# AI4quantum/qiskit-gym

Hardware: AMD Instinct MI355X
Metric: env-steps/sec (whole node), CliffordGym 16q x 65536 envs/GPU; bit-exact vs CPU (higher is better)
Workload: dtype u32

## Files before the change

### qiskit_gym_amd/csrc/kernels_pauli_tile.hip

```cpp
#include <algorithm>
#include <cstdlib>
#include <cstring>

#include "device_common.hpp"
#include "pauli_common.hpp"

namespace qg {

static uint64_t ptile_program(const qg_gate &g) {
    const uint32_t a = (uint32_t)g.q0, b = g.kind >= QG_CX ? (uint32_t)g.q1 : (uint32_t)g.q0;
    struct Mop { uint32_t kind; bool swapped; };
    Mop mops[3] = {{M_NOP, false}, {M_NOP, false}, {M_NOP, false}};
    switch (g.kind) {
    case QG_H: mops[0] = {M_H, false}; break;
    case QG_S: mops[0] = {M_S, false}; break;
    case QG_SDG: mops[0] = mops[1] = mops[2] = {M_S, false}; break;
    case QG_SX: mops[0] = {M_SX, false}; break;
    case QG_SXDG: mops[0] = mops[1] = mops[2] = {M_SX, false}; break;
    case QG_CX: mops[0] = {M_CNOT, false}; break;
    case QG_CZ: mops[0] = {M_H, true}; mops[1] = {M_CNOT, false}; mops[2] = {M_H, true}; break;
    case QG_SWAP: mops[0] = {M_CNOT, false}; mops[1] = {M_CNOT, true}; mops[2] = {M_CNOT, false}; break;
    }
    uint32_t row[4] = {1, 2, 4, 8};
    auto X = [&](bool second) -> uint32_t & { return row[(second && a != b) ? 2 : 0]; };
// ... 1112 lines not shown
    const uint64_t w = row < N ? wx : wz;
    const uint32_t extra = row < N ? ex : ez;
    if (a.format == QG_FMT_PACKED) {
        reinterpret_cast<uint64_t *>(a.out)[env * a.out_stride + row] = w;
        return;
    }
    if (a.format == QG_FMT_I64) {
        int64_t *o = reinterpret_cast<int64_t *>(a.out) + env * a.out_stride + (uint64_t)row * cols;
        for (uint32_t c = 0; c < D; ++c) o[c] = (int64_t)((w >> c) & 1ull);
        for (uint32_t c = D; c < cols; ++c) o[c] = (int64_t)((extra >> (c - D)) & 1u);
    } else {
        int8_t *o = reinterpret_cast<int8_t *>(a.out) + env * a.out_stride + (uint64_t)row * cols;
        for (uint32_t c = 0; c < D; ++c) o[c] = (int8_t)((w >> c) & 1ull);
        for (uint32_t c = D; c < cols; ++c) o[c] = (int8_t)((extra >> (c - D)) & 1u);
    }
}


struct PTGenArgs {
    StepArgs s;
    const uint8_t *pairs;
    const uint32_t *dvals;
    const uint32_t *doff;
    const uint8_t *cx_pairs;
    uint32_t nd, n_cx;
    uint64_t seed;
    uint32_t difficulty, pauli_difficulty, max_paulis;
    float decay;
    int32_t depth_value;
    uint32_t only_done;
    const uint32_t *list;
    uint32_t *list_count;
    uint32_t n_pairs;
    uint32_t gen_grid;
    uint32_t tree_grid;
    uint32_t *count_out;
    uint32_t tree;
    unsigned long long *tree_kclk;
    const uint64_t *mask;
    uint32_t mask_words, mask_epoch;
    uint32_t *count_pub;
};
constexpr uint32_t PT_CX_LDS = plan::PAULI_CX_LDS;
using plan::pauli_tree_takes;

constexpr uint64_t PT_STREAM_LABELS = 0x7061756Cull, PT_STREAM_TABLEAU = 0x7461626Cull;
struct PTStream {
    uint64_t seed, env, k;
    const uint64_t *pre = nullptr;
    uint32_t n_pre = 0;
    __device__ uint64_t at(uint64_t i) const { return (pre && i < n_pre) ? pre[i] : rng_draw(seed, env, i); }
    __device__ uint64_t next() { return at(k++); }
    __device__ uint32_t range(uint32_t n) { return (uint32_t)__umul64hi(next(), (uint64_t)n); }
    __device__ float f32() { return (float)(next() >> 40) * (1.0f / 16777216.0f); }
};

struct PTGenTables {
    alignas(4) uint8_t cx[2 * PT_CX_LDS];
    uint32_t dvals[32], doff[33];
    alignas(4) uint8_t pairs[2 * 496];
};
__device__ inline bool pt_gen_tables_load(const PTGenArgs &ga, PTGenTables &t) {
    const bool cx_in_lds = ga.n_cx <= PT_CX_LDS;
    const uint32_t nd = ga.nd < 32u ? ga.nd : 32u;
    const uint32_t n_pairs = ga.n_pairs < 496u ? ga.n_pairs : 496u;
    const uint32_t cx_words = cx_in_lds ? (2u * ga.n_cx + 3u) / 4u : 0u, pair_words = (2u * n_pairs + 3u) / 4u;
    const uint32_t *cxw = reinterpret_cast<const uint32_t *>(ga.cx_pairs), *pw = reinterpret_cast<const uint32_t *>(ga.pairs);
    uint32_t *t_cx = reinterpret_cast<uint32_t *>(t.cx), *t_pairs = reinterpret_cast<uint32_t *>(t.pairs);
    constexpr uint32_t CX_PER = 8, PAIR_PER = 4;
    uint32_t cv[CX_PER], pv[PAIR_PER];
    const uint32_t dv = threadIdx.x < nd ? ga.dvals[threadIdx.x] : 0u, df = threadIdx.x <= nd ? ga.doff[threadIdx.x] : 0u;
#pragma unroll
    for (uint32_t k = 0; k < CX_PER; ++k) {
        const uint32_t i = threadIdx.x + k * blockDim.x;
// ... 223 lines not shown
    s.bad = (uint32_t)__ballot(q_lane && (X != ix || Z != iz));
    uint32_t n_removed = 0, fault = 0;
    uint64_t rem_pos[(RM + 7) / 8];
#pragma unroll
    for (int i = 0; i < (RM + 7) / 8; ++i) rem_pos[i] = 0;
    pt_clean<NQ, RM>(s, n_removed, fault, SolLog{nullptr, 0}, rem_pos);
    const bool solved = pt_solved<NQ, RM>(s);
    if (q_lane) L::store_qubit(tile, le, lane, X, Z);
    if constexpr (L::COMPACT) {
        if (q_lane) pt_store_xz<NQ, RM>(tile, le, s, lane);
        if (lane == 0) pt_store_rotmeta<NQ, RM>(tile, le, s, true);
    } else {
        if (lane == 0) pt_store_rotations<NQ, RM>(tile, le, s, ~0u, ~0u, true);
    }
    if (lane != 0) return;
    pt_store_meta<NQ, RM>(tile, le, s);
    a.depth[env] = ga.depth_value;
    a.success[env] = (uint8_t)solved;
    a.reward[env] = solved ? 1.0f : 0.0f;
    a.done[env] = (uint8_t)(ga.depth_value == 0 || solved);
    a.inverted[env] = 0;
    a.error[env] = fault;
    a.sol_len[env * 2] = 0;
    a.sol_len[env * 2 + 1] = 0;
    if (a.layers) {
        const LayerRec lay = layer_rec(a.layers, env, (2 * N + 2));
        for (uint32_t i = 0; i < 2 * N; ++i) lay[i] = -1;
        lay[2 * N] = 0;
        lay[2 * N + 1] = 0;
    }
}

template <int NQ, int RM>
__device__ __forceinline__ bool ptile_generate_body(const PTGenArgs &ga, uint32_t vblock) {
    const StepArgs &a = ga.s;
    __shared__ uint64_t lds_tab[2 * NQ][QG_WAVE];
    __shared__ PTGenTables tb;
    const uint64_t tid = (uint64_t)vblock * QG_WAVE + threadIdx.x;
    __shared__ uint32_t mask_part[64 + 1 + 5];
    uint32_t count = ga.list ? ga.list_count[0] : 0u;
    if (ga.mask) {
        const bool published = ga.tree != 0;
        count = published ? *ga.count_pub : 0u;
        if (published && (pauli_tree_takes(count, ga.difficulty, a.B, ga.n_cx) || (tid & ~(uint64_t)(QG_WAVE - 1)) >= count)) return false;
        DoneMaskShare share;
        done_mask_load<64>(ga.mask, a.B, ga.mask_words, share);
        count = *done_mask_hint(ga.mask, a.B) != ga.mask_epoch ? 0u : done_mask_scan<64>(share, mask_part);
        if ((tid & ~(uint64_t)(QG_WAVE - 1)) >= count) return false;
    } else if (ga.list && ((ga.tree && pauli_tree_takes(count, ga.difficulty, a.B, ga.n_cx)) || (tid & ~(uint64_t)(QG_WAVE - 1)) >= count)) {
        return false;
    }
    const bool cx_in_lds = pt_gen_tables_load(ga, tb);
    __builtin_amdgcn_fence(__ATOMIC_RELEASE, "wavefront");
    __builtin_amdgcn_wave_barrier();
    uint64_t env = tid;
    if (ga.mask) {
        if (tid >= count) return true;
        env = done_mask_nth<64>(ga.mask, ga.mask_words, mask_part, (uint32_t)tid);
    } else if (ga.list) {
        if (tid >= count) return true;
        env = ga.list[tid];
    } else {
        if (env >= a.B) return true;
        if (ga.only_done && !a.done[env]) return true;
    }
    const uint32_t L = threadIdx.x & (QG_WAVE - 1);
    const uint32_t N = a.N;
    const uint64_t base_seed = ga.seed + QG_CLOCK_SEED_STRIDE * clock_of(a.clock);
    PTStream rng{base_seed ^ PT_STREAM_LABELS, a.env_base + env, 0};
    PTState<NQ, RM> s;
    (void)pt_gen_labels<NQ, RM>(ga, tb, rng, s, N);

#pragma unroll
    for (int j = 0; j < NQ; ++j) {
        lds_tab[j][L] = (uint32_t)j < N ? 1ull << j : 0ull;
        lds_tab[NQ + j][L] = (uint32_t)j < N ? (1ull << N) << j : 0ull;
    }
    if (ga.difficulty != 0 && ga.n_cx != 0) {
        const uint64_t tseed = base_seed ^ PT_STREAM_TABLEAU;
        for (uint32_t it0 = 0; it0 < ga.difficulty; it0 += 4) {
            uint64_t d1[4], d2[4];
#pragma unroll
            for (uint32_t j = 0; j < 4; ++j) {
                d1[j] = rng_draw(tseed, rng.env, 2ull * (it0 + j));
                d2[j] = rng_draw(tseed, rng.env, 2ull * (it0 + j) + 1ull);
            }
#pragma unroll
            for (uint32_t j = 0; j < 4; ++j) {
                if (it0 + j >= ga.difficulty) break;
                const float r = (float)(d1[j] >> 40) * (1.0f / 16777216.0f);
                if (r > 0.3f) {
                    const uint32_t k = (uint32_t)__umul64hi(d2[j], (uint64_t)ga.n_cx);
                    const uint32_t q0 = cx_in_lds ? tb.cx[2 * k] : ga.cx_pairs[2 * k], q1 = cx_in_lds ? tb.cx[2 * k + 1] : ga.cx_pairs[2 * k + 1];
                    const uint64_t x0 = lds_tab[q0][L], z1 = lds_tab[NQ + q1][L];
                    lds_tab[q1][L] ^= x0;
                    lds_tab[NQ + q0][L] ^= z1;
                } else if (r > 0.15f) {
                    const uint32_t q = (uint32_t)__umul64hi(d2[j], (uint64_t)N);
                    const uint64_t x = lds_tab[q][L], z = lds_tab[NQ + q][L];
                    lds_tab[q][L] = z;
                    lds_tab[NQ + q][L] = x;
                } else {
                    const uint32_t q = (uint32_t)__umul64hi(d2[j], (uint64_t)N);
                    lds_tab[NQ + q][L] ^= lds_tab[q][L];
                }
            }
        }
    }
#pragma unroll
    for (int j = 0; j < NQ; ++j) {
        s.X[j] = lds_tab[j][L];
        s.Z[j] = lds_tab[NQ + j][L];
    }
    pt_gen_finish<NQ, RM>(ga, s, env, N);
    return true;
}
template <int NQ, int RM>
__global__ __launch_bounds__(64) void ptile_generate_kernel(PTGenArgs ga) {
    KernelClock kclk(ga.s.kclk, ga.s.kclk_waves);
    if (ga.mask && ga.tree) {
        const uint32_t count = *ga.count_pub;
        if (!count || pauli_tree_takes(count, ga.difficulty, ga.s.B, ga.n_cx)) return;
    }
    const uint32_t total = (uint32_t)((ga.s.B + QG_WAVE - 1) / QG_WAVE);
    for (uint32_t vblock = blockIdx.x; vblock < total; vblock += gridDim.x) {
        if (!ptile_generate_body<NQ, RM>(ga, vblock)) break;
        __builtin_amdgcn_wave_barrier();
    }
}

constexpr uint32_t PT_TREE_THREADS = QG_TREE_THREADS + QG_WAVE;
template <int NQ, int RM>
__global__ __launch_bounds__(PT_TREE_THREADS) void ptile_reset_tree_kernel(PTGenArgs ga) {
    KernelClock kclk(ga.tree_kclk, ga.s.kclk_waves);
    const StepArgs &a = ga.s;
    constexpr int R = 2 * NQ;
    __shared__ uint64_t prod[4][64];
    __shared__ RowopMasks64 tree_gates[4][QG_WAVE];
    __shared__ PTGenTables tb;
    __shared__ uint64_t rows_out[64];
    __shared__ uint64_t pre_draws[QG_TREE_THREADS];
    uint32_t count;
    __shared__ uint32_t mask_part[PT_TREE_THREADS + 2 + PT_TREE_THREADS / 64];
    DoneMaskShare share;
    uint32_t opaque_zero, first_v = 0;
    asm("v_mov_b32 %0, 0" : "=v"(opaque_zero));
    if (ga.mask) {
        first_v = done_mask_hint(ga.mask, a.B)[opaque_zero];
        done_mask_load<PT_TREE_THREADS>(ga.mask, a.B, ga.mask_words, share);
    } else {
        first_v = ga.list_count[opaque_zero];
    }
    asm volatile("" ::: "memory");
    (void)pt_gen_tables_load(ga, tb);
    if (ga.mask) {
        count = (uint32_t)__builtin_amdgcn_readfirstlane((int)first_v) != ga.mask_epoch ? 0u : done_mask_scan<PT_TREE_THREADS>(share, mask_part);
        if (blockIdx.x == 0 && threadIdx.x == 0) *ga.count_pub = count;
    } else {
        count = (uint32_t)__builtin_amdgcn_readfirstlane((int)first_v);
    }
    if (ga.count_out && blockIdx.x == 0 && threadIdx.x == 0) *ga.count_out = count;
    if (threadIdx.x == 0) phase_stamp(ga.tree_kclk, a.kclk_waves, 0);
    if (!pauli_tree_takes(count, ga.difficulty, a.B, ga.n_cx)) return;
    const uint32_t N = a.N, lane = threadIdx.x & (QG_WAVE - 1), wave = threadIdx.x >> 6;
    __shared__ uint32_t prod_ready[4];
    if (threadIdx.x < 4u) prod_ready[threadIdx.x] = 0u;
    uint32_t prod_seq = 0;
    for (uint32_t item = blockIdx.x; item < count; item += gridDim.x) {
    if (item != blockIdx.x) __syncthreads();
    const uint64_t env = !ga.mask ? ga.list[item]
                       : item == blockIdx.x ? done_mask_find<PT_TREE_THREADS>(ga.mask, ga.mask_words, share, mask_part, item)
                                            : done_mask_nth<PT_TREE_THREADS>(ga.mask, ga.mask_words, mask_part, item);
    const uint64_t base_seed = ga.seed + QG_CLOCK_SEED_STRIDE * clock_of(a.clock), renv = a.env_base + env;
    PTStream rng{base_seed ^ PT_STREAM_LABELS, renv, 0};
    if (threadIdx.x < QG_TREE_THREADS) pre_draws[threadIdx.x] = rng_draw(rng.seed, rng.env, threadIdx.x);
    __syncthreads();
    rng.pre = pre_draws;
    rng.n_pre = QG_TREE_THREADS;
    if ((threadIdx.x & 63u) == 0 && (wave == 0u || wave == 4u)) phase_stamp(ga.tree_kclk, a.kclk_waves, wave == 0u ? 1u : 2u);
    if (wave == 4u) {
        PTState<NQ, RM> s;
        (void)pt_gen_labels_wave<NQ, RM>(ga, tb, rng, s, N);
        phase_stamp(ga.tree_kclk, a.kclk_waves, 3);
        __syncthreads();
        phase_stamp(ga.tree_kclk, a.kclk_waves, 5);
        pt_gen_finish_wave<NQ, RM>(ga, s, env, N, rows_out);
        phase_stamp(ga.tree_kclk, a.kclk_waves, 6);
        continue;
    }
    const uint32_t n_cx = ga.n_cx;
    const uint8_t *cx = tb.cx;
    const uint64_t tseed = base_seed ^ PT_STREAM_TABLEAU;
    uint64_t row = 0;
    const bool finisher = scramble_tree64_ops<R>(
        ga.difficulty, row, prod, tree_gates,
        [N](uint32_t k) -> uint64_t { const uint32_t j = k < (uint32_t)NQ ? k : k - (uint32_t)NQ; return j < N ? (k < (uint32_t)NQ ? 1ull << j : (1ull << N) << j) : 0ull; },
        [=](uint32_t it) -> uint32_t {
            const uint64_t d1 = rng_draw(tseed, renv, 2ull * it), d2 = rng_draw(tseed, renv, 2ull * it + 1ull);
// ... 164 lines not shown
    ObsArgs a;
    memset(&a, 0, sizeof a);
    a.state = v->state;
    a.B = v->B;
    a.N = v->N;
    a.D = 2 * v->N;
    a.obs_rows = 2 * v->N;
    a.obs_cols = 2 * v->N + (uint32_t)std::max(v->cfg.max_rotations, 1);
    a.format = QG_FMT_U8;
    if (!a.B) return hipSuccess;
    PTObsArgs pa;
    fill_obs(v, a, pa);
    hipLaunchKernelGGL(ptile_rowwords_kernel, dim3(grid_for(a.B * 2ull * a.N / 2, 256)), dim3(256), 0, s, pa, reinterpret_cast<uint64_t *>(out_dev));
    return hipGetLastError();
}

hipError_t ptile_observe_typed(qg_vec *v, void *out_dev, int out_dtype, hipStream_t s) {
    ObsArgs a;
    memset(&a, 0, sizeof a);
    a.state = v->state;
    a.B = v->B;
    a.N = v->N;
    a.D = 2 * v->N;
    a.obs_rows = 2 * v->N;
    a.obs_cols = 2 * v->N + (uint32_t)std::max(v->cfg.max_rotations, 1);
    a.format = QG_FMT_U8;
    if (!a.B) return hipSuccess;
    return ptile_dense_via_words(v, a, out_dev, out_dtype, s);
}


template <int NQ, int RM>
static hipError_t pt_launch_generate(const PTGenArgs &pa, hipStream_t s) {
    if (pa.tree) {
        const uint64_t blocks = pa.tree_grid;
        if (blocks) hipLaunchKernelGGL((ptile_reset_tree_kernel<NQ, RM>), dim3((unsigned)blocks), dim3(PT_TREE_THREADS), 0, s, pa);
    }
    const unsigned all = grid_for(pa.s.B, 64);
    hipLaunchKernelGGL((ptile_generate_kernel<NQ, RM>), dim3(pa.gen_grid && pa.gen_grid < all ? pa.gen_grid : all), dim3(64), 0, s, pa);
    return hipGetLastError();
}
static hipError_t ptile_generate(const qg_vec *v, const PTGenArgs &pa, hipStream_t s) { PT_DISPATCH(pt_launch_generate) }

int ptile_reset_seeded(qg_vec *v, uint64_t seed, bool only_done, hipStream_t s, bool from_mask) {
    const uint32_t n = v->N;
    if (!v->d_gen_tables) {
        std::vector<uint8_t> cx;
        std::vector<std::vector<uint32_t>> adj(n);
        for (const qg_gate &g : v->gates)
            if (g.kind == QG_CX) {
                cx.push_back((uint8_t)g.q0);
                cx.push_back((uint8_t)g.q1);
                auto add = [&](uint32_t a, uint32_t b) { if (std::find(adj[a].begin(), adj[a].end(), b) == adj[a].end()) adj[a].push_back(b); };
                add((uint32_t)g.q0, (uint32_t)g.q1);
                add((uint32_t)g.q1, (uint32_t)g.q0);
            }
        std::vector<std::vector<int>> dist(n, std::vector<int>(n, -1));
        for (uint32_t st = 0; st < n; ++st) {
            std::vector<uint32_t> q{st};
            dist[st][st] = 0;
            for (size_t h = 0; h < q.size(); ++h)
                for (uint32_t w : adj[q[h]])
                    if (dist[st][w] < 0) { dist[st][w] = dist[st][q[h]] + 1; q.push_back(w); }
        }
        std::vector<uint8_t> pairs;
        std::vector<uint32_t> dvals, doff;
        for (int d = 1; d < (int)n; ++d) {
            const size_t before = pairs.size();
            for (uint32_t a = 0; a < n; ++a)
                for (uint32_t b = a + 1; b < n; ++b)
                    if (dist[a][b] == d) { pairs.push_back((uint8_t)a); pairs.push_back((uint8_t)b); }
            if (pairs.size() != before) { dvals.push_back((uint32_t)d); doff.push_back((uint32_t)(before / 2)); }
// ... 19 lines not shown
    a.state = v->state;
    a.depth = v->depth;
    a.reward = v->reward;
    a.done = v->done;
    a.success = v->success;
    a.inverted = v->inverted;
    a.error = v->error;
    a.sol_len = v->sol_len;
    a.layers = v->layers;
    a.B = v->B;
    a.N = n;
    const uint8_t *base = reinterpret_cast<const uint8_t *>(v->d_gen_tables);
    ga.dvals = reinterpret_cast<const uint32_t *>(base + v->gen_off[0]);
    ga.doff = reinterpret_cast<const uint32_t *>(base + v->gen_off[1]);
    ga.pairs = base + v->gen_off[2];
    ga.cx_pairs = base + v->gen_off[3];
    ga.nd = v->gen_nd;
    ga.n_cx = v->gen_ncx;
    ga.n_pairs = v->gen_npairs;
    ga.seed = seed;
    a.clock = v->clock_dev;
    a.env_base = v->env_base;
    ga.difficulty = (uint32_t)v->difficulty;
    ga.pauli_difficulty = (uint32_t)(v->difficulty / std::max(v->cfg.pauli_diff_scale, 1));
    ga.max_paulis = v->plan.rmax_generate;
    ga.decay = v->cfg.num_qubits_decay;
    const int64_t d = (int64_t)v->cfg.depth_slope * v->difficulty;
    ga.depth_value = (int32_t)std::min<int64_t>(d, v->cfg.max_depth);
    ga.only_done = only_done ? 1u : 0u;
    if (only_done && from_mask && v->done_mask[0]) {
        ga.mask = v->done_mask[v->dl.cur()];
        ga.mask_words = (uint32_t)done_mask_words(v->B);
        ga.mask_epoch = v->dl.epoch();
        ga.count_pub = v->mask_count;
        ga.tree = (ga.difficulty >= plan::TREE_MIN_DRAWS && v->B / 32u >= 1u && pauli_tree_takes(1u, ga.difficulty, v->B, ga.n_cx)) ? 1u : 0u;
    } else if (only_done && v->done_list && v->B > QG_COMPACT_MIN_ENVS) {
        HIP_TRY(compact_done(v->done, v->B, v->done_list, v->done_list + v->B, s));
        ga.list = v->done_list;
        ga.list_count = v->done_list + v->B;
        ga.tree = (ga.difficulty >= plan::TREE_MIN_DRAWS && v->B / 32u >= 1u && pauli_tree_takes(1u, ga.difficulty, v->B, ga.n_cx)) ? 1u : 0u;
    }
    if (ga.tree) {
        ga.tree_grid = reset_tree_grid(v, (uint32_t)(v->B / 32u));
        ga.gen_grid = reset_second_grid(v, [](uint32_t count, const qg_vec *h) -> bool {
            return pauli_tree_takes(count, (uint32_t)h->difficulty, h->B, h->gen_ncx);
        });
        ga.count_out = v->count_seen;
        ga.tree_kclk = kernel_clock_slot(v);
    }
    a.kclk = kernel_clock_slot(v);
    a.kclk_waves = v->kclk_waves;
    HIP_TRY(ptile_generate(v, ga, s));
    return QG_OK;
}

int ptile_upload(qg_vec *v, const HostNet &h, bool do_clean, int32_t depth_value, hipStream_t s) {
    const uint32_t N = v->N, NQ = v->plan.pt_nq, RM = v->plan.pt_rm;
    const bool compact = v->plan.pauli_compact;
    const size_t QB = compact ? 768 : 1024, RB = compact ? 512 : 1024, tile_bytes = NQ * QB + RM * RB + (RM > 16 ? 3072 : 1024);
    std::vector<uint8_t> img(v->plan.state_bytes, 0);
    for (uint64_t e = 0; e < v->B; ++e) {
        uint8_t *tile = img.data() + (e >> 6) * tile_bytes;
        const uint32_t lane = (uint32_t)(e & 63);
        for (uint32_t q = 0; q < N; ++q) {
            const uint64_t x = h.tab[(e * N + q) * 2], z = h.tab[(e * N + q) * 2 + 1];
            if (compact) {
                uint32_t g[3] = {(uint32_t)x, ((uint32_t)(x >> 32) & 0xFFFFu) | ((uint32_t)z << 16), (uint32_t)(z >> 16)};
                memcpy(tile + q * QB + lane * 12, g, 12);
            } else {
                uint32_t g[4] = {(uint32_t)x, (uint32_t)(x >> 32), (uint32_t)z, (uint32_t)(z >> 32)};
                memcpy(tile + q * QB + lane * 16, g, 16);
            }
        }
        if (compact) {
            uint8_t *rb = tile + NQ * QB;
            auto byte_at = [&](uint32_t b) -> uint8_t & { return rb[(b >> 3) * RB + lane * 8 + (b & 7u)]; };
            uint32_t wp[5] = {0, 0, 0, 0, 0}, plo = 0, phi = 0;
            for (uint32_t k = 0; k < v->plan.rmax; ++k) {
                const PauliRot &r = h.rot[e * v->plan.rmax + k];
                for (uint32_t q = 0; q < N; ++q) {
                    byte_at(2 * q) |= (uint8_t)(((r.x >> q) & 1u) << k);
                    byte_at(2 * q + 1) |= (uint8_t)(((r.z >> q) & 1u) << k);
                }
// ... 55 lines not shown
```

### qiskit_gym_amd/csrc/qgym_api.cpp

```cpp
#include <atomic>
#include <hip/hip_runtime.h>

#include <algorithm>
#include <cmath>
#include <cctype>
#include <cstdarg>
#include <cstdio>
#include <cstdlib>
#include <cstring>
#include <memory>
#include <string>
#include <vector>

#include "pauli_common.hpp"

namespace qg {

static thread_local std::string g_err;

int set_error(int code, const char *fmt, ...) {
    char buf[512];
    va_list ap;
    va_start(ap, fmt);
    vsnprintf(buf, sizeof buf, fmt, ap);
// ... 206 lines not shown
    while (b < e && isspace((unsigned char)name[b])) ++b;
    while (e > b && isspace((unsigned char)name[e - 1])) --e;
    name = name.substr(b, e - b);
    std::string key = name;
    for (auto &ch : key) ch = (char)tolower((unsigned char)ch);
    for (size_t i = 0; i < n; ++i)
        if (idx[i] < 0) return set_error(QG_ERR_TYPE, "Gate indices must be non-negative integers (usize)");
    static const char *one_q[] = {"h", "s", "sdg", "sx", "sxdg"};
    static const char *two_q[] = {"cx", "cz", "swap"};
    for (int k = 0; k < 5; ++k)
        if (key == one_q[k]) {
            if (n != 1) return set_error(QG_ERR_INVALID, "Gate `%s` expects 1 index, got %zu", name.c_str(), n);
            out->kind = k;
            out->q0 = (int32_t)idx[0];
            out->q1 = 0;
            return QG_OK;
        }
    for (int k = 0; k < 3; ++k)
        if (key == two_q[k]) {
            if (n != 2) return set_error(QG_ERR_INVALID, "Gate `%s` expects 2 indices, got %zu", name.c_str(), n);
            out->kind = 5 + k;
            out->q0 = (int32_t)idx[0];
            out->q1 = (int32_t)idx[1];
            return QG_OK;
        }
    return set_error(QG_ERR_INVALID, "Unknown gate name `%s`. Allowed: H, S, Sdg, SX, SXdg, CX, CZ, SWAP", name.c_str());
}


static int vec_free_buffers(qg_vec *v) {
    void *ptrs[] = {v->state, v->own_depth ? v->depth : nullptr, v->own_reward ? v->reward : nullptr,
                    v->own_done ? v->done : nullptr, v->own_success ? v->success : nullptr, v->inverted, v->own_error ? v->error : nullptr, v->sol,
                    v->sol_len, v->layers, v->d_gates, v->d_descs, v->scratch, v->d_prog,
                    v->d_qubit_perms, v->d_act_perms, v->perm_idx, v->d_gen_tables, v->d_nonsymp, v->bad, v->done_list, v->done_list_alt, v->done_list_spare, v->done_mask[0], v->done_mask[1], v->mask_count, v->d_rowops, v->embed_dump, v->host_in, v->host_obs, v->fault_scratch, v->d_twist_obs, v->twist_words};
    for (void *p : ptrs)
        if (p) (void)hipFree(p);
    drop_graphs(v);
    if (v->capture_stream) (void)hipStreamDestroy(v->capture_stream);
    if (v->fault_word) (void)hipHostFree(v->fault_word);
    if (v->count_seen) (void)hipHostFree(v->count_seen);
    return 0;
}

static int drop_done_list(qg_vec *v, hipStream_t s) { return zero_list_length(v, v->done_list, v->dl.drop(), s); }

static void fill_init_args(const qg_vec *v, InitArgs &a) {
    memset(&a, 0, sizeof a);
    a.tree_grid = plan::tree_grid(v->B);
    a.state = v->state;
    a.depth = v->depth;
    a.reward = v->reward;
    a.done = v->done;
    a.success = v->success;
    a.inverted = v->inverted;
    a.error = v->error;
    a.sol_len = v->sol_len;
    a.layers = v->layers;
    a.layers_len = v->layers_len;
    a.gates = v->d_gates;
    a.B = v->B;
    a.D = v->plan.D;
    a.N = v->N;
    a.num_actions = (uint32_t)v->gates.size();
    a.clock = v->clock_dev;
    a.env_base = v->env_base;
    a.bad = v->bad;
    a.rowops = v->d_rowops;
// ... 105 lines not shown
#define HIP_TRY_V(expr)                                                                            \
    do {                                                                                           \
        hipError_t _e = (expr);                                                                    \
        if (_e != hipSuccess) {                                                                    \
            (void)hipGetLastError();                                                               \
            return fail(set_error(QG_ERR_DEVICE, "%s failed: %s", #expr, hipGetErrorString(_e)));  \
        }                                                                                          \
    } while (0)

    HIP_TRY_V(hipMalloc(&p->state, hp.state_bytes));
    HIP_TRY_V(hipMemset(p->state, 0, hp.state_bytes));
    HIP_TRY_V(hipMalloc(&p->depth, sizeof(int32_t) * batch));
    HIP_TRY_V(hipMalloc(&p->reward, sizeof(float) * batch));
    HIP_TRY_V(hipMalloc(&p->done, batch));
    HIP_TRY_V(hipMalloc(&p->success, batch));
    HIP_TRY_V(hipMalloc(&p->inverted, batch));
    if (hp.has_bad)
        HIP_TRY_V(hipMalloc(&p->bad, plan::bad_word_bytes(hp) * batch));
    if (hp.has_done_list) {
        HIP_TRY_V(hipMalloc(&p->done_list, sizeof(uint32_t) * (batch + 2)));
        HIP_TRY_V(hipMemset(p->done_list + batch, 0, 2 * sizeof(uint32_t)));
    }
    if (hp.has_done_list && plan::is_tile(hp)) {
        HIP_TRY_V(hipMalloc(&p->done_list_spare, sizeof(uint32_t) * (batch + 2)));
        HIP_TRY_V(hipMemset(p->done_list_spare + batch, 0, 2 * sizeof(uint32_t)));
    }
    if (plan::reset_step_fusable(hp)) {
        HIP_TRY_V(hipMalloc(&p->done_list_alt, sizeof(uint32_t) * (batch + 2)));
        HIP_TRY_V(hipMemset(p->done_list_alt + batch, 0, 2 * sizeof(uint32_t)));
    }
    if (hp.has_done_list) {
        HIP_TRY_V(hipHostMalloc((void **)&p->count_seen, sizeof(uint32_t), hipHostMallocMapped));
        *p->count_seen = 0xFFFFFFFFu;
        if (hp.layout != LAYOUT_TILE) {
            HIP_TRY_V(hipMalloc(&p->mask_count, 2 * sizeof(uint32_t)));
            HIP_TRY_V(hipMemset(p->mask_count, 0, 2 * sizeof(uint32_t)));
        }
        for (auto &m : p->done_mask) {
            HIP_TRY_V(hipMalloc(&m, done_mask_bytes(batch)));
            HIP_TRY_V(hipMemset(m, 0, done_mask_bytes(batch)));
        }
    }
    HIP_TRY_V(hipMalloc(&p->error, sizeof(uint32_t) * batch));
    HIP_TRY_V(hipMalloc(&p->sol_len, sizeof(int32_t) * 2 * batch));
    if (cfg->track_solution) {
        p->sol_cap = (uint32_t)std::max(cfg->max_depth, 1);
        if (hp.layout == LAYOUT_PAULI) p->sol_cap += hp.rmax;
        HIP_TRY_V(hipMalloc(&p->sol, sizeof(uint32_t) * (size_t)p->sol_cap * batch));
    }
    if (layers) {
        p->layers_len = 2 * N + 2;
        HIP_TRY_V(hipMalloc(&p->layers, sizeof(int32_t) * (size_t)p->layers_len * (((size_t)batch + 63) & ~(size_t)63)));
    }
    (void)device_compute_units(device);
    uint32_t group_bytes[plan::GROUP_TABLE_DWORDS] = {};
    if (hp.layout == LAYOUT_TILE) plan::gate_group_bytes(&table[0].ops, sizeof(GateEntry) / sizeof(uint32_t), n_gates, hp.has_z, group_bytes);
    HIP_TRY_V(hipMalloc(&p->d_gates, sizeof(GateEntry) * table.size() + sizeof group_bytes));
    HIP_TRY_V(hipMalloc(&p->d_descs, sizeof(uint32_t) * descs.size()));
    HIP_TRY_V(hipMemcpy(p->d_gates, table.data(), sizeof(GateEntry) * table.size(), hipMemcpyHostToDevice));
    HIP_TRY_V(hipMemcpy(p->d_gates + n_gates, group_bytes, sizeof group_bytes, hipMemcpyHostToDevice));
    HIP_TRY_V(hipMemcpy(p->d_descs, descs.data(), sizeof(uint32_t) * descs.size(), hipMemcpyHostToDevice));
    if (plan::is_tile(hp)) {
        std::vector<uint32_t> rowops(table.size(), 0u);
        auto slot = [&](uint32_t row) { return hp.has_z ? (row < N ? 2 * row : 2 * (row - N) + 1) : row; };
        for (size_t i = 0; i < n_gates; ++i) {
            const uint32_t ops = gate_ops(cfg->env_kind, gates[i], N);
            uint32_t out = 0;
            for (int k = 0; k < 2; ++k) {
                const uint32_t op = (ops >> (14 * k)) & 0x3FFFu, type = (op >> 12) & 3u;
                if (type != OP_NONE) out |= make_op(type, slot(op & 63u), slot((op >> 6) & 63u)) << (14 * k);
// ... 230 lines not shown
        HIP_TRY(hipStreamSynchronize(s));
    }
    return QG_OK;
}

static int do_reset(qg_vec *v, const int32_t *actions_dev, uint64_t seed, hipStream_t s, bool only_done = false) {
    QG_ON_DEVICE(v);
    const bool trusted = v->dl.enter(session_of(s));
    if (int rc = only_done ? QG_OK : drop_done_list(v, s)) return rc;
    if (only_done && v->plan.layout == LAYOUT_PAULI) return ptile_reset_seeded(v, seed, true, s, v->dl.pauli_reset_consumes(trusted));
    if (v->plan.layout == LAYOUT_PAULI) {
        if (actions_dev) return set_error(QG_ERR_UNSUPPORTED, "PauliEnv reset draws a whole target, not `difficulty` actions: use qg_vec_reset(seed) or qg_vec_pauli_reset_from");
        return pauli_reset_seeded(v, seed, s);
    }
    if (v->gates.empty() && v->difficulty)
        return set_error(QG_ERR_PANIC, "reset with an empty gateset (the reference panics in Uniform::new(0, 0))");
    InitArgs ia;
    fill_reset_done_args(v, seed, ia);
    ia.actions = actions_dev;
    ia.only_done = only_done ? 1u : 0u;
    if (only_done && v->done_list) {
        const DoneListState::Consume use = v->dl.reset_consumes(trusted);
        if (use.compact) HIP_TRY(compact_done(v->done, v->B, v->done_list, v->done_list + v->B, s));
        ia.list = v->done_list;
        ia.list_count = v->done_list + v->B;
        if (plan::is_tile(v->plan) && v->count_seen) {
            ia.count_out = v->count_seen;
            ia.tree_grid = reset_tree_grid(v, plan::tree_grid(v->B));
        }
        if (use.mask && v->done_mask[0]) {
            ia.mask = v->done_mask[v->dl.cur()];
            ia.mask_words = (uint32_t)done_mask_words(v->B);
            ia.mask_epoch = v->dl.epoch();
            ia.count_pub = v->mask_count;
        }
        ia.coop = plan::reset_coop_allowed(actions_dev != nullptr, v->B, v->d_rowops != nullptr) ? 1u : 0u;
        ia.flags_current = 1u;
        if (v->plan.layout == LAYOUT_TILE) ia.dense = v->dense;
        if (v->done_list_spare) ia.zero_count = v->done_list_spare + v->B;
    }
    if (!only_done) v->maybe_nonsymplectic = false;
    HIP_TRY(launch_init(v, ia, s));
    if (ia.zero_count) std::swap(v->done_list, v->done_list_spare);
    if (v->dense && !ia.dense) return dense_refresh(v, s);
    return QG_OK;
}

int qg_vec_set_clock(qg_vec *v, const uint64_t *clock_dev) {
    if (!v) return set_error(QG_ERR_INVALID, "null argument");
    QG_ON_DEVICE(v);
    HIP_TRY(hipDeviceSynchronize());
    v->clock_dev = clock_dev;
    drop_graphs(v);
    return QG_OK;
}

int qg_vec_set_kernel_clock(qg_vec *v, uint64_t *slots_dev, size_t n_slots, uint32_t waves_per_slot) {
    if (!v || (n_slots && (!slots_dev || !waves_per_slot))) return set_error(QG_ERR_INVALID, "null argument");
    if ((uintptr_t)slots_dev & 15u) return set_error(QG_ERR_INVALID, "kernel clock slots must be 16-byte aligned");
    drop_graphs(v);
    v->kclk = n_slots ? reinterpret_cast<unsigned long long *>(slots_dev) : nullptr;
    v->kclk_cap = n_slots;
    v->kclk_waves = n_slots ? waves_per_slot : 0u;
    v->kclk_next = 0;
    return QG_OK;
}

// ... 605 lines not shown
        hipMemcpy(len.data(), v->sol_len, len.size() * sizeof(int32_t), hipMemcpyDeviceToHost) != hipSuccess ||
        hipMemcpy(log.data(), v->sol, log.size() * sizeof(uint32_t), hipMemcpyDeviceToHost) != hipSuccess) {
        (void)hipGetLastError();
        return set_error(QG_ERR_DEVICE, "solution copy failed");
    }
    for (size_t e = 0; e < v->B; ++e) lens[e] = (int64_t)decode_solution(v, log.data() + e, v->B, &len[2 * e], out ? out + e * cap : nullptr, cap);
    return QG_OK;
}

}

namespace qg {
uint64_t session_of(hipStream_t s) {
    hipStreamCaptureStatus cs = hipStreamCaptureStatusNone;
    unsigned long long id = 0;
    if (s) (void)hipStreamGetCaptureInfo(s, &cs, &id);
    return cs == hipStreamCaptureStatusNone ? 0ull : (id ? (uint64_t)id : ~0ull);
}
int zero_list_length(const qg_vec *v, uint32_t *list, bool needed, hipStream_t s) {
    if (needed) HIP_TRY(hipMemsetAsync(list + v->B, 0, 2 * sizeof(uint32_t), s));
    return QG_OK;
}
int bind_error(qg_vec *v, uint32_t *error_dev) {
    if (!v || !error_dev) return set_error(QG_ERR_INVALID, "null argument");
    QG_ON_DEVICE(v);
    HIP_TRY(hipDeviceSynchronize());
    HIP_TRY(hipMemcpy(error_dev, v->error, sizeof(uint32_t) * v->B, hipMemcpyDefault));
    if (v->own_error) (void)hipFree(v->error);
    v->error = error_dev;
    v->own_error = false;
    drop_graphs(v);
    return QG_OK;
}
uint32_t reset_second_grid(const qg_vec *v, bool is_tree_list_of_that_length(uint32_t, const qg_vec *)) {
    const uint32_t seen = v->count_seen ? *(volatile const uint32_t *)v->count_seen : 0xFFFFFFFFu;
    return (seen != 0xFFFFFFFFu && (seen == 0 || is_tree_list_of_that_length(seen, v))) ? 32u : 0u;
}

int dense_refresh(qg_vec *v, hipStream_t s) {
    ObsArgs oa;
    fill_obs_args(v, oa, v->dense, QG_FMT_U8, (size_t)v->plan.D * v->plan.D);
    HIP_TRY(launch_export(v, oa, s));
    return QG_OK;
}
void fill_reset_done_args(const qg_vec *v, uint64_t seed, InitArgs &ia) {
    fill_init_args(v, ia);
    ia.mode = 2;
    ia.n_draws = (uint32_t)v->difficulty;
    ia.seed = seed;
    ia.only_done = 1u;
    ia.depth_value = (int32_t)std::min<int64_t>((int64_t)v->cfg.depth_slope * v->difficulty, v->cfg.max_depth);
}
}
```

### qiskit_gym_amd/csrc/qgym_host.hpp

```cpp
#pragma once

#include <string.h>
#include <string>
#include <vector>

#include "qgym_done_list.hpp"
#include "qgym_internal.hpp"
#include "qgym_plan.hpp"

namespace qg {

struct GraphKey {
    const void *actions;
    const void *coins;
    const void *rewards;
    const void *dones;
    size_t T;
    int dtype;
    size_t period;
    uint32_t flags;
    uint64_t env_base;
    const void *dense;
    bool operator==(const GraphKey &o) const {
        return actions == o.actions && coins == o.coins && rewards == o.rewards && dones == o.dones && T == o.T &&
// ... 58 lines not shown
    unsigned long long *kclk = nullptr;
    size_t kclk_cap = 0;
    uint32_t kclk_waves = 0;
    mutable size_t kclk_next = 0;

    void *state = nullptr;
    int32_t *depth = nullptr;
    float *reward = nullptr;
    uint8_t *done = nullptr;
    uint8_t *success = nullptr;
    uint8_t *inverted = nullptr;
    uint32_t *error = nullptr;
    uint32_t *sol = nullptr;
    int32_t *sol_len = nullptr;
    int32_t *layers = nullptr;
    qg::GateEntry *d_gates = nullptr;
    uint32_t *d_descs = nullptr;
    uint32_t sol_cap = 0;
    uint32_t layers_len = 0;
    void *scratch = nullptr;
    size_t scratch_bytes = 0;
    void *host_in = nullptr;
    void *host_obs = nullptr;
    size_t host_obs_bytes = 0;
    uint32_t *count_seen = nullptr;
    uint32_t *fault_word = nullptr;
    uint32_t *fault_scratch = nullptr;
    uint32_t *bad = nullptr;
    uint32_t *d_rowops = nullptr;
    uint32_t *done_list = nullptr;
    uint32_t *done_list_alt = nullptr;
    uint32_t *done_list_spare = nullptr;
    uint64_t *done_mask[2] = {nullptr, nullptr};
    uint32_t *mask_count = nullptr;
    qg::DoneListState dl;
    int8_t *dense = nullptr;
    uint32_t *d_nonsymp = nullptr;
    void *embed_dump = nullptr;
    bool maybe_nonsymplectic = false;
    bool own_reward = true, own_done = true, own_success = true, own_depth = true;
    bool own_error = true;

    void *d_prog = nullptr;
    void *d_gen_tables = nullptr;
    uint32_t gen_nd = 0, gen_ncx = 0, gen_npairs = 0, gen_off[4] = {0, 0, 0, 0};
    uint8_t *d_qubit_perms = nullptr;
    int32_t *d_act_perms = nullptr;
    uint32_t *perm_idx = nullptr;
    const int32_t *perm_in = nullptr;
    uint32_t n_perms = 0;
    bool perm_draw = false;
    uint64_t observe_counter = 0;

    bool twists_done = false;
    std::vector<std::vector<int64_t>> obs_perms, act_perms;
    int32_t *d_twist_obs = nullptr;
    void *twist_words = nullptr;
    size_t twist_words_bytes = 0;

    std::vector<qg::CachedGraph> graphs;
    hipStream_t capture_stream = nullptr;
};

namespace qg {
inline bool same_ctor(const qg_vec *a, const qg_vec *b) {
    return a->device == b->device && memcmp(&a->cfg, &b->cfg, sizeof a->cfg) == 0 && a->gates.size() == b->gates.size() &&
           (a->gates.empty() || memcmp(a->gates.data(), b->gates.data(), a->gates.size() * sizeof(qg_gate)) == 0);
}
int ensure_scratch(qg_vec *v, size_t bytes);
inline void destroy_graph(CachedGraph &g) {
    if (g.exec) (void)hipGraphExecDestroy(g.exec);
    if (g.graph) (void)hipGraphDestroy(g.graph);
}
inline void drop_graphs(qg_vec *v) {
    for (auto &g : v->graphs) destroy_graph(g);
    v->graphs.clear();
}
uint64_t session_of(hipStream_t s);
int zero_list_length(const qg_vec *v, uint32_t *list, bool needed, hipStream_t s);
void fill_step_args(const qg_vec *v, StepArgs &a);
int bind_error(qg_vec *v, uint32_t *error_dev);
uint32_t reset_second_grid(const qg_vec *v, bool is_tree_list_of_that_length(uint32_t, const qg_vec *));
uint32_t reset_tree_grid(const qg_vec *v, uint32_t most);
unsigned long long *kernel_clock_slot(const qg_vec *v);
int dense_refresh(qg_vec *v, hipStream_t s);
void fill_reset_done_args(const qg_vec *v, uint64_t seed, InitArgs &ia);
void compute_qubit_and_action_perms(uint32_t N, const std::vector<qg_gate> &gates, std::vector<std::vector<int64_t>> &qubit_perms,
                                    std::vector<std::vector<int64_t>> &act_perms);
void build_twists(const qg_vec *v, std::vector<std::vector<int64_t>> &obs_perms, std::vector<std::vector<int64_t>> &act_perms);
int twist_expand_impl(const void *packed_dev, int word_bytes, uint64_t batch, uint32_t rows, uint32_t cols, const int32_t *obs_perms_dev,
                      uint32_t n_twists, const int32_t *twist_idx_dev, void *out_dev, int out_dtype, hipStream_t s);
int twist_words_impl(const void *packed_dev, int word_bytes, uint64_t batch, uint32_t rows, uint32_t cols, const int32_t *obs_perms_dev,
                     uint32_t n_twists, const int32_t *twist_idx_dev, uint64_t *out_dev, uint32_t rows_out, hipStream_t s);
int pauli_alloc(qg_vec *v);
int pauli_init_identity(qg_vec *v, hipStream_t s);
int pauli_set_state(qg_vec *v, const void *states, int format, size_t stride, int on_device, hipStream_t s);
int pauli_reset_from(qg_vec *v, const uint8_t *tableaus, const char *labels, const int32_t *n_rot, hipStream_t s);
int pauli_reset_seeded(qg_vec *v, uint64_t seed, hipStream_t s);
hipError_t pauli_step(const qg_vec *v, const StepArgs &a, hipStream_t s);
hipError_t pauli_export(const qg_vec *v, const ObsArgs &a, hipStream_t s);
}
```

Baseline: 26.11 billion.

## Fold per-env generate walk into reset tree kernel, dropping second launch

When the tree path is selected, the reset tree kernel now also handles the case where the tree is not taken: it walks the done list or mask itself, using a union of LDS between the tree scratch and a per-wave tableau, instead of publishing a count and launching a second generate kernel. This removes one kernel launch per reset, the count_pub global handshake and the host-side second-grid heuristic. The cost is a heavier tree kernel with more LDS and a waves_per_eu attribute, and the walk runs only on the first wave of blocks up to count/64, which may give less parallelism than the old separate generate grid.

After: 26.08 billion, median of 2. No clear change (-0.1%).

```diff
diff --git a/qiskit_gym_amd/csrc/kernels_pauli_tile.hip b/qiskit_gym_amd/csrc/kernels_pauli_tile.hip
--- a/qiskit_gym_amd/csrc/kernels_pauli_tile.hip
+++ b/qiskit_gym_amd/csrc/kernels_pauli_tile.hip
@@ -1168,14 +1168,12 @@
     const uint32_t *list;
     uint32_t *list_count;
     uint32_t n_pairs;
-    uint32_t gen_grid;
     uint32_t tree_grid;
     uint32_t *count_out;
     uint32_t tree;
     unsigned long long *tree_kclk;
     const uint64_t *mask;
     uint32_t mask_words, mask_epoch;
-    uint32_t *count_pub;
 };
 constexpr uint32_t PT_CX_LDS = plan::PAULI_CX_LDS;
 using plan::pauli_tree_takes;
@@ -1465,38 +1463,8 @@
 }
 
 template <int NQ, int RM>
-__device__ __forceinline__ bool ptile_generate_body(const PTGenArgs &ga, uint32_t vblock) {
+__device__ __forceinline__ void ptile_generate_env(const PTGenArgs &ga, const PTGenTables &tb, uint64_t (*lds_tab)[QG_WAVE], bool cx_in_lds, uint64_t env) {
     const StepArgs &a = ga.s;
-    __shared__ uint64_t lds_tab[2 * NQ][QG_WAVE];
-    __shared__ PTGenTables tb;
-    const uint64_t tid = (uint64_t)vblock * QG_WAVE + threadIdx.x;
-    __shared__ uint32_t mask_part[64 + 1 + 5];
-    uint32_t count = ga.list ? ga.list_count[0] : 0u;
-    if (ga.mask) {
-        const bool published = ga.tree != 0;
-        count = published ? *ga.count_pub : 0u;
-        if (published && (pauli_tree_takes(count, ga.difficulty, a.B, ga.n_cx) || (tid & ~(uint64_t)(QG_WAVE - 1)) >= count)) return false;
-        DoneMaskShare share;
-        done_mask_load<64>(ga.mask, a.B, ga.mask_words, share);
-        count = *done_mask_hint(ga.mask, a.B) != ga.mask_epoch ? 0u : done_mask_scan<64>(share, mask_part);
-        if ((tid & ~(uint64_t)(QG_WAVE - 1)) >= count) return false;
-    } else if (ga.list && ((ga.tree && pauli_tree_takes(count, ga.difficulty, a.B, ga.n_cx)) || (tid & ~(uint64_t)(QG_WAVE - 1)) >= count)) {
-        return false;
-    }
-    const bool cx_in_lds = pt_gen_tables_load(ga, tb);
-    __builtin_amdgcn_fence(__ATOMIC_RELEASE, "wavefront");
-    __builtin_amdgcn_wave_barrier();
-    uint64_t env = tid;
-    if (ga.mask) {
-        if (tid >= count) return true;
-        env = done_mask_nth<64>(ga.mask, ga.mask_words, mask_part, (uint32_t)tid);
-    } else if (ga.list) {
-        if (tid >= count) return true;
-        env = ga.list[tid];
-    } else {
-        if (env >= a.B) return true;
-        if (ga.only_done && !a.done[env]) return true;
-    }
     const uint32_t L = threadIdx.x & (QG_WAVE - 1);
     const uint32_t N = a.N;
     const uint64_t base_seed = ga.seed + QG_CLOCK_SEED_STRIDE * clock_of(a.clock);
@@ -1546,15 +1514,44 @@
         s.Z[j] = lds_tab[NQ + j][L];
     }
     pt_gen_finish<NQ, RM>(ga, s, env, N);
+}
+
+template <int NQ, int RM>
+__device__ __forceinline__ bool ptile_generate_body(const PTGenArgs &ga, uint32_t vblock) {
+    const StepArgs &a = ga.s;
+    __shared__ uint64_t lds_tab[2 * NQ][QG_WAVE];
+    __shared__ PTGenTables tb;
+    const uint64_t tid = (uint64_t)vblock * QG_WAVE + threadIdx.x;
+    __shared__ uint32_t mask_part[64 + 1 + 5];
+    uint32_t count = ga.list ? ga.list_count[0] : 0u;
+    if (ga.mask) {
+        DoneMaskShare share;
+        done_mask_load<64>(ga.mask, a.B, ga.mask_words, share);
+        count = *done_mask_hint(ga.mask, a.B) != ga.mask_epoch ? 0u : done_mask_scan<64>(share, mask_part);
+        if ((tid & ~(uint64_t)(QG_WAVE - 1)) >= count) return false;
+    } else if (ga.list && (tid & ~(uint64_t)(QG_WAVE - 1)) >= count) {
+        return false;
+    }
+    const bool cx_in_lds = pt_gen_tables_load(ga, tb);
+    __builtin_amdgcn_fence(__ATOMIC_RELEASE, "wavefront");
+    __builtin_amdgcn_wave_barrier();
+    uint64_t env = tid;
+    if (ga.mask) {
+        if (tid >= count) return true;
+        env = done_mask_nth<64>(ga.mask, ga.mask_words, mask_part, (uint32_t)tid);
+    } else if (ga.list) {
+        if (tid >= count) return true;
+        env = ga.list[tid];
+    } else {
+        if (env >= a.B) return true;
+        if (ga.only_done && !a.done[env]) return true;
+    }
+    ptile_generate_env<NQ, RM>(ga, tb, lds_tab, cx_in_lds, env);
     return true;
 }
 template <int NQ, int RM>
 __global__ __launch_bounds__(64) void ptile_generate_kernel(PTGenArgs ga) {
     KernelClock kclk(ga.s.kclk, ga.s.kclk_waves);
-    if (ga.mask && ga.tree) {
-        const uint32_t count = *ga.count_pub;
-        if (!count || pauli_tree_takes(count, ga.difficulty, ga.s.B, ga.n_cx)) return;
-    }
     const uint32_t total = (uint32_t)((ga.s.B + QG_WAVE - 1) / QG_WAVE);
     for (uint32_t vblock = blockIdx.x; vblock < total; vblock += gridDim.x) {
         if (!ptile_generate_body<NQ, RM>(ga, vblock)) break;
@@ -1563,16 +1560,51 @@
 }
 
 constexpr uint32_t PT_TREE_THREADS = QG_TREE_THREADS + QG_WAVE;
-template <int NQ, int RM>
-__global__ __launch_bounds__(PT_TREE_THREADS) void ptile_reset_tree_kernel(PTGenArgs ga) {
+struct PTTreeLds {
+    uint64_t prod[4][64];
+    RowopMasks64 tree_gates[4][QG_WAVE];
+    uint64_t rows_out[64];
+    uint64_t pre_draws[QG_TREE_THREADS];
+    uint32_t prod_ready[4];
+};
+template <int NQ>
+union PTResetLds {
+    PTTreeLds tree;
+    uint64_t walk_tab[2 * NQ][QG_WAVE];
+};
+using PTGenArgsSegment = const __attribute__((address_space(4))) PTGenArgs *;
+template <int NQ, int RM>
+__device__ __noinline__ void ptile_tree_walk(PTGenArgsSegment args, uint32_t count, const PTGenTables *tb_lds, const uint32_t *mask_part_lds,
+                                             uint64_t (*tab_lds)[QG_WAVE]) {
+    const uint64_t args_v = (uint64_t)args;
+    const uint32_t args_lo = (uint32_t)__builtin_amdgcn_readfirstlane((int)(uint32_t)args_v), args_hi = (uint32_t)__builtin_amdgcn_readfirstlane((int)(uint32_t)(args_v >> 32));
+    const PTGenArgs &ga = *(const PTGenArgs *)(PTGenArgsSegment)(((uint64_t)args_hi << 32) | args_lo);
+    const PTGenTables &tb = *(const PTGenTables *)(const __attribute__((address_space(3))) PTGenTables *)tb_lds;
+    const uint32_t *mask_part = (const uint32_t *)(const __attribute__((address_space(3))) uint32_t *)mask_part_lds;
+    uint64_t (*tab)[QG_WAVE] = (uint64_t (*)[QG_WAVE])(__attribute__((address_space(3))) uint64_t (*)[QG_WAVE])tab_lds;
+    count = (uint32_t)__builtin_amdgcn_readfirstlane((int)count);
+    const uint32_t vblocks = (count + QG_WAVE - 1u) / QG_WAVE;
+    for (uint32_t vblock = blockIdx.x; vblock < vblocks; vblock += gridDim.x) {
+        const uint32_t i = vblock * QG_WAVE + threadIdx.x;
+        if (i < count) {
+            const uint64_t env = ga.mask ? done_mask_nth<PT_TREE_THREADS>(ga.mask, ga.mask_words, mask_part, i) : ga.list[i];
+            ptile_generate_env<NQ, RM>(ga, tb, tab, true , env);
+        }
+        __builtin_amdgcn_wave_barrier();
+    }
+}
+template <int NQ, int RM>
+__global__ __launch_bounds__(PT_TREE_THREADS) __attribute__((amdgpu_waves_per_eu(RM > 16 ? 4 : 5))) void ptile_reset_tree_kernel(PTGenArgs ga) {
     KernelClock kclk(ga.tree_kclk, ga.s.kclk_waves);
     const StepArgs &a = ga.s;
     constexpr int R = 2 * NQ;
-    __shared__ uint64_t prod[4][64];
-    __shared__ RowopMasks64 tree_gates[4][QG_WAVE];
+    __shared__ PTResetLds<NQ> lds;
+    uint64_t (&prod)[4][64] = lds.tree.prod;
+    RowopMasks64 (&tree_gates)[4][QG_WAVE] = lds.tree.tree_gates;
+    uint64_t (&rows_out)[64] = lds.tree.rows_out;
+    uint64_t (&pre_draws)[QG_TREE_THREADS] = lds.tree.pre_draws;
+    uint32_t (&prod_ready)[4] = lds.tree.prod_ready;
     __shared__ PTGenTables tb;
-    __shared__ uint64_t rows_out[64];
-    __shared__ uint64_t pre_draws[QG_TREE_THREADS];
     uint32_t count;
     __shared__ uint32_t mask_part[PT_TREE_THREADS + 2 + PT_TREE_THREADS / 64];
     DoneMaskShare share;
@@ -1588,15 +1620,18 @@
     (void)pt_gen_tables_load(ga, tb);
     if (ga.mask) {
         count = (uint32_t)__builtin_amdgcn_readfirstlane((int)first_v) != ga.mask_epoch ? 0u : done_mask_scan<PT_TREE_THREADS>(share, mask_part);
-        if (blockIdx.x == 0 && threadIdx.x == 0) *ga.count_pub = count;
     } else {
         count = (uint32_t)__builtin_amdgcn_readfirstlane((int)first_v);
     }
     if (ga.count_out && blockIdx.x == 0 && threadIdx.x == 0) *ga.count_out = count;
     if (threadIdx.x == 0) phase_stamp(ga.tree_kclk, a.kclk_waves, 0);
-    if (!pauli_tree_takes(count, ga.difficulty, a.B, ga.n_cx)) return;
+    if (!pauli_tree_takes(count, ga.difficulty, a.B, ga.n_cx)) {
+        if (blockIdx.x >= (count + QG_WAVE - 1u) / QG_WAVE) return;
+        __syncthreads();
+        if (threadIdx.x < QG_WAVE) ptile_tree_walk<NQ, RM>((PTGenArgsSegment)__builtin_amdgcn_kernarg_segment_ptr(), count, &tb, mask_part, lds.walk_tab);
+        return;
+    }
     const uint32_t N = a.N, lane = threadIdx.x & (QG_WAVE - 1), wave = threadIdx.x >> 6;
-    __shared__ uint32_t prod_ready[4];
     if (threadIdx.x < 4u) prod_ready[threadIdx.x] = 0u;
     uint32_t prod_seq = 0;
     for (uint32_t item = blockIdx.x; item < count; item += gridDim.x) {
@@ -1827,12 +1862,11 @@
 
 template <int NQ, int RM>
 static hipError_t pt_launch_generate(const PTGenArgs &pa, hipStream_t s) {
-    if (pa.tree) {
-        const uint64_t blocks = pa.tree_grid;
-        if (blocks) hipLaunchKernelGGL((ptile_reset_tree_kernel<NQ, RM>), dim3((unsigned)blocks), dim3(PT_TREE_THREADS), 0, s, pa);
-    }
-    const unsigned all = grid_for(pa.s.B, 64);
-    hipLaunchKernelGGL((ptile_generate_kernel<NQ, RM>), dim3(pa.gen_grid && pa.gen_grid < all ? pa.gen_grid : all), dim3(64), 0, s, pa);
+    if (pa.tree && pa.tree_grid) {
+        hipLaunchKernelGGL((ptile_reset_tree_kernel<NQ, RM>), dim3(pa.tree_grid), dim3(PT_TREE_THREADS), 0, s, pa);
+        return hipGetLastError();
+    }
+    hipLaunchKernelGGL((ptile_generate_kernel<NQ, RM>), dim3(grid_for(pa.s.B, 64)), dim3(64), 0, s, pa);
     return hipGetLastError();
 }
 static hipError_t ptile_generate(const qg_vec *v, const PTGenArgs &pa, hipStream_t s) { PT_DISPATCH(pt_launch_generate) }
@@ -1918,7 +1952,6 @@
         ga.mask = v->done_mask[v->dl.cur()];
         ga.mask_words = (uint32_t)done_mask_words(v->B);
         ga.mask_epoch = v->dl.epoch();
-        ga.count_pub = v->mask_count;
         ga.tree = (ga.difficulty >= plan::TREE_MIN_DRAWS && v->B / 32u >= 1u && pauli_tree_takes(1u, ga.difficulty, v->B, ga.n_cx)) ? 1u : 0u;
     } else if (only_done && v->done_list && v->B > QG_COMPACT_MIN_ENVS) {
         HIP_TRY(compact_done(v->done, v->B, v->done_list, v->done_list + v->B, s));
@@ -1928,13 +1961,11 @@
     }
     if (ga.tree) {
         ga.tree_grid = reset_tree_grid(v, (uint32_t)(v->B / 32u));
-        ga.gen_grid = reset_second_grid(v, [](uint32_t count, const qg_vec *h) -> bool {
-            return pauli_tree_takes(count, (uint32_t)h->difficulty, h->B, h->gen_ncx);
-        });
         ga.count_out = v->count_seen;
         ga.tree_kclk = kernel_clock_slot(v);
-    }
-    a.kclk = kernel_clock_slot(v);
+    } else {
+        a.kclk = kernel_clock_slot(v);
+    }
     a.kclk_waves = v->kclk_waves;
     HIP_TRY(ptile_generate(v, ga, s));
     return QG_OK;
diff --git a/qiskit_gym_amd/csrc/qgym_api.cpp b/qiskit_gym_amd/csrc/qgym_api.cpp
--- a/qiskit_gym_amd/csrc/qgym_api.cpp
+++ b/qiskit_gym_amd/csrc/qgym_api.cpp
@@ -262,7 +262,7 @@
     void *ptrs[] = {v->state, v->own_depth ? v->depth : nullptr, v->own_reward ? v->reward : nullptr,
                     v->own_done ? v->done : nullptr, v->own_success ? v->success : nullptr, v->inverted, v->own_error ? v->error : nullptr, v->sol,
                     v->sol_len, v->layers, v->d_gates, v->d_descs, v->scratch, v->d_prog,
-                    v->d_qubit_perms, v->d_act_perms, v->perm_idx, v->d_gen_tables, v->d_nonsymp, v->bad, v->done_list, v->done_list_alt, v->done_list_spare, v->done_mask[0], v->done_mask[1], v->mask_count, v->d_rowops, v->embed_dump, v->host_in, v->host_obs, v->fault_scratch, v->d_twist_obs, v->twist_words};
+                    v->d_qubit_perms, v->d_act_perms, v->perm_idx, v->d_gen_tables, v->d_nonsymp, v->bad, v->done_list, v->done_list_alt, v->done_list_spare, v->done_mask[0], v->done_mask[1], v->d_rowops, v->embed_dump, v->host_in, v->host_obs, v->fault_scratch, v->d_twist_obs, v->twist_words};
     for (void *p : ptrs)
         if (p) (void)hipFree(p);
     drop_graphs(v);
@@ -434,10 +434,6 @@
     if (hp.has_done_list) {
         HIP_TRY_V(hipHostMalloc((void **)&p->count_seen, sizeof(uint32_t), hipHostMallocMapped));
         *p->count_seen = 0xFFFFFFFFu;
-        if (hp.layout != LAYOUT_TILE) {
-            HIP_TRY_V(hipMalloc(&p->mask_count, 2 * sizeof(uint32_t)));
-            HIP_TRY_V(hipMemset(p->mask_count, 0, 2 * sizeof(uint32_t)));
-        }
         for (auto &m : p->done_mask) {
             HIP_TRY_V(hipMalloc(&m, done_mask_bytes(batch)));
             HIP_TRY_V(hipMemset(m, 0, done_mask_bytes(batch)));
@@ -734,7 +730,6 @@
             ia.mask = v->done_mask[v->dl.cur()];
             ia.mask_words = (uint32_t)done_mask_words(v->B);
             ia.mask_epoch = v->dl.epoch();
-            ia.count_pub = v->mask_count;
         }
         ia.coop = plan::reset_coop_allowed(actions_dev != nullptr, v->B, v->d_rowops != nullptr) ? 1u : 0u;
         ia.flags_current = 1u;
@@ -1406,11 +1401,6 @@
     drop_graphs(v);
     return QG_OK;
 }
-uint32_t reset_second_grid(const qg_vec *v, bool is_tree_list_of_that_length(uint32_t, const qg_vec *)) {
-    const uint32_t seen = v->count_seen ? *(volatile const uint32_t *)v->count_seen : 0xFFFFFFFFu;
-    return (seen != 0xFFFFFFFFu && (seen == 0 || is_tree_list_of_that_length(seen, v))) ? 32u : 0u;
-}
-
 int dense_refresh(qg_vec *v, hipStream_t s) {
     ObsArgs oa;
     fill_obs_args(v, oa, v->dense, QG_FMT_U8, (size_t)v->plan.D * v->plan.D);
diff --git a/qiskit_gym_amd/csrc/qgym_host.hpp b/qiskit_gym_amd/csrc/qgym_host.hpp
--- a/qiskit_gym_amd/csrc/qgym_host.hpp
+++ b/qiskit_gym_amd/csrc/qgym_host.hpp
@@ -114,7 +114,6 @@
     uint32_t *done_list_alt = nullptr;
     uint32_t *done_list_spare = nullptr;
     uint64_t *done_mask[2] = {nullptr, nullptr};
-    uint32_t *mask_count = nullptr;
     qg::DoneListState dl;
     int8_t *dense = nullptr;
     uint32_t *d_nonsymp = nullptr;
@@ -162,7 +161,6 @@
 int zero_list_length(const qg_vec *v, uint32_t *list, bool needed, hipStream_t s);
 void fill_step_args(const qg_vec *v, StepArgs &a);
 int bind_error(qg_vec *v, uint32_t *error_dev);
-uint32_t reset_second_grid(const qg_vec *v, bool is_tree_list_of_that_length(uint32_t, const qg_vec *));
 uint32_t reset_tree_grid(const qg_vec *v, uint32_t most);
 unsigned long long *kernel_clock_slot(const qg_vec *v);
 int dense_refresh(qg_vec *v, hipStream_t s);
```
